# eladhoffer/convNet.pytorch

Hardware: NVIDIA H100
Metric: ResNet-50 images/sec (training step, synthetic 224x224) (higher is better)
Workload: dtype bf16

## Files before the change

convnet/pytorch_b200/csrc/conv.cu:

```cuda
#include "common.cuh"
#include "host.h"
#include <stdlib.h>
#include <utility>

namespace b200 {

constexpr int kMaxStages = 8;
constexpr int kMaxTaps = 32;
constexpr int kThreads = 384;
constexpr int kConsumers = 256;
constexpr int kProducerWarp = 8;
constexpr int kTileM = 128;
constexpr int kStatReplicas = 16;

struct TapEntry {
  uint16_t off_w, off_h;
  uint16_t b_tap;
  uint16_t pad_;
};

struct IgemmParams {
  int M_total;
  int I, J;
  int trav;
// ... 749 lines not shown
            "smem=%d\n",
            p.M_total, L.SC, L.Nout, L.ntaps, L.os, p.block_n, p.n_tiles, p.m_tiles, p.ck, L.ntaps * p.c_chunks,
            p.num_stages, p.tma_store, p.plain_a, p.b_stationary, p.own_ntile, p.out_fp32, L.bias != nullptr,
            L.res != nullptr, p.act, L.stats != nullptr, grid, max_tiles, smem_bytes);
  }
  b200::launch(kfn, grid, kThreads, smem_bytes, stream, tmA, tmB, tmC, tmR, p);
  B200_CHECK_LAUNCH("conv_igemm_kernel");
  return B200_OK;
}

static int check_desc(const b200_conv_desc* d) {
  B200_REQUIRE(d != nullptr, B200_ERR_INVALID, "conv: null descriptor");
  B200_REQUIRE(d->N > 0 && d->H > 0 && d->W > 0 && d->C > 0 && d->K > 0 && d->R > 0 && d->S > 0 && d->P > 0 &&
                   d->Q > 0 && d->stride >= 1 && d->stride <= 8,
               B200_ERR_INVALID, "conv: bad descriptor N=%d H=%d W=%d C=%d K=%d R=%d S=%d P=%d Q=%d stride=%d", d->N,
               d->H, d->W, d->C, d->K, d->R, d->S, d->P, d->Q, d->stride);
  B200_REQUIRE(d->R * d->S <= kMaxTaps, B200_ERR_UNSUPPORTED, "conv: %dx%d filter exceeds %d taps", d->R, d->S,
               kMaxTaps);
  B200_REQUIRE((d->x_pixel_stride == 0 && d->x_row_stride == 0 && d->x_image_stride == 0) ||
                   (d->x_pixel_stride > 0 && d->x_pixel_stride % 8 == 0 && d->x_row_stride % 8 == 0 &&
                    d->x_image_stride % 8 == 0 && d->x_row_stride > 0 && d->x_image_stride > 0),
               B200_ERR_INVALID, "conv: x strides must all be 0 (dense) or positive multiples of 8 elements");
  B200_REQUIRE(d->window == 0 || (d->window % 64 == 0 && d->C == d->K && d->C % d->window == 0 && d->x_pixel_stride == 0),
               B200_ERR_UNSUPPORTED, "conv: window %d needs C == K, C %% window == 0 (C=%d K=%d)", d->window, d->C, d->K);
  return B200_OK;
}

}

using namespace b200;

extern "C" int b200_conv_fprop(const b200_conv_desc* d, const void* x, const void* w, void* y,
                               const b200_epilogue* ep, b200_stream_t stream) {
  int rc = check_desc(d);
  if (rc) return rc;
  B200_REQUIRE(x && w && y, B200_ERR_INVALID, "conv_fprop: null pointer");
  B200_REQUIRE(d->C % 8 == 0, B200_ERR_UNSUPPORTED, "conv_fprop: C=%d must be a multiple of 8 (pad the input)", d->C);
  if (d->stride == 1 && d->pad_h == d->pad_w && d->P == d->H + 2 * d->pad_h - d->R + 1 &&
      d->Q == d->W + 2 * d->pad_w - d->S + 1 && d->x_pixel_stride == 0 && (!ep || !ep->out_fp32) &&
      !(ep && ep->bias && ep->bn_stats_workspace) && (d->window == 0 || d->window == 64) &&
      halo_eligible(d->P, d->Q, d->C, d->K, d->R, d->S, d->pad_h)) {
    return launch_halo(x, w, y, ep ? ep->residual : nullptr, ep ? ep->bias : nullptr, d->N, d->P, d->Q, d->C, d->K,
                       d->R, d->S, d->pad_h, 0, ep ? ep->act : 0,
                       (ep && ep->bn_stats_workspace) ? reinterpret_cast<double*>(ep->bn_stats_workspace) : nullptr,
                       (cudaStream_t)stream, d->window);
  }
  IgemmLaunch L;
  memset(&L, 0, sizeof(L));
  L.src = x; L.Nimg = d->N; L.SH = d->H; L.SW = d->W; L.SC = d->C;
  L.s_pix = d->x_pixel_stride; L.s_row = d->x_row_stride; L.s_img = d->x_image_stride;
  L.wmat = w; L.Nout = d->K; L.wtaps = d->R * d->S;
  L.I = d->P; L.J = d->Q; L.trav = d->stride; L.lower_w = -d->pad_w; L.lower_h = -d->pad_h;
  L.ntaps = d->R * d->S;
  for (int r = 0; r < d->R; ++r)
    for (int s = 0; s < d->S; ++s) {
      TapEntry& t = L.taps[r * d->S + s];
      t.off_w = (uint16_t)s; t.off_h = (uint16_t)r; t.b_tap = (uint16_t)(r * d->S + s); t.pad_ = 0;
    }
  L.out = y; L.OH = d->P; L.OW = d->Q; L.os = 1; L.oh0 = 0; L.ow0 = 0; L.ldo = d->K;
  L.res = ep ? ep->residual : nullptr;
  L.bias = ep ? ep->bias : nullptr;
  L.act = ep ? ep->act : 0;
  L.out_fp32 = ep ? ep->out_fp32 : 0;
  L.stats = (ep && ep->bn_stats_workspace) ? reinterpret_cast<double*>(ep->bn_stats_workspace) : nullptr;
  L.window = d->window;
  return launch_igemm(L, (cudaStream_t)stream);
}

extern "C" int b200_conv_dgrad(const b200_conv_desc* d, const void* dy, const void* wt, void* dx,
                               const void* residual, b200_stream_t stream_) {
  int rc = check_desc(d);
  if (rc) return rc;
  cudaStream_t stream = (cudaStream_t)stream_;
  B200_REQUIRE(dy && wt && dx, B200_ERR_INVALID, "conv_dgrad: null pointer");
  B200_REQUIRE(d->K % 8 == 0, B200_ERR_UNSUPPORTED, "conv_dgrad: K=%d must be a multiple of 8", d->K);
  const int st = d->stride;
  B200_REQUIRE(st == 1 || st == 2, B200_ERR_UNSUPPORTED, "conv_dgrad: stride %d unsupported", st);
  if (d->R == 3 && d->S == 3 && st == 1 && d->pad_h == 1 && d->pad_w == 1 && d->P == d->H && d->Q == d->W &&
      (d->window == 0 || d->window == 64) && halo_eligible(d->H, d->W, d->K, d->C, 3, 3, 1)) {
    return launch_halo(dy, wt, dx, residual, nullptr, d->N, d->H, d->W, d->K, d->C, 3, 3, 1, 1, 0, nullptr, stream,
                       d->window);
  }
  bool any_empty = false;
  for (int ph = 0; ph < st; ++ph)
    for (int pw = 0; pw < st; ++pw) {
      int nr = 0, ns = 0;
      for (int r = 0; r < d->R; ++r) if (((ph + d->pad_h - r) % st + st) % st == 0) ++nr;
      for (int s = 0; s < d->S; ++s) if (((pw + d->pad_w - s) % st + st) % st == 0) ++ns;
      if (nr * ns == 0 && (d->H - ph + st - 1) / st > 0 && (d->W - pw + st - 1) / st > 0) any_empty = true;
    }
  if (any_empty) {
    B200_REQUIRE(residual == nullptr, B200_ERR_UNSUPPORTED,
                 "conv_dgrad: residual add with an empty stride class is unsupported");
    cudaError_t e = cudaMemsetAsync(dx, 0, (size_t)d->N * d->H * d->W * d->C * 2, stream);
    B200_REQUIRE(e == cudaSuccess, B200_ERR_CUDA, "conv_dgrad: memset failed: %s", cudaGetErrorString(e));
    count_launch();
  }
  for (int ph = 0; ph < st; ++ph)
    for (int pw = 0; pw < st; ++pw) {
      const int I = (d->H - ph + st - 1) / st;
      const int J = (d->W - pw + st - 1) / st;
      if (I <= 0 || J <= 0) continue;
      IgemmLaunch L;
      memset(&L, 0, sizeof(L));
      int dh[kMaxTaps], dwv[kMaxTaps], rr[kMaxTaps], ss[kMaxTaps];
      int nr = 0, ns = 0;
      for (int r = 0; r < d->R; ++r) {
        const int v = ph + d->pad_h - r;
        if (((v % st) + st) % st == 0) { dh[nr] = (v - (((v % st) + st) % st)) / st; rr[nr] = r; ++nr; }
      }
      for (int s = 0; s < d->S; ++s) {
        const int v = pw + d->pad_w - s;
        if (((v % st) + st) % st == 0) { dwv[ns] = (v - (((v % st) + st) % st)) / st; ss[ns] = s; ++ns; }
      }
      if (nr * ns == 0) continue;
      int lo_h = dh[0], lo_w = dwv[0];
      for (int i = 1; i < nr; ++i) lo_h = dh[i] < lo_h ? dh[i] : lo_h;
      for (int i = 1; i < ns; ++i) lo_w = dwv[i] < lo_w ? dwv[i] : lo_w;
      L.ntaps = nr * ns;
      for (int a = 0; a < nr; ++a)
        for (int b = 0; b < ns; ++b) {
          TapEntry& t = L.taps[a * ns + b];
          t.off_h = (uint16_t)(dh[a] - lo_h);
          t.off_w = (uint16_t)(dwv[b] - lo_w);
          t.b_tap = (uint16_t)(rr[a] * d->S + ss[b]);
          t.pad_ = 0;
        }
      L.src = dy; L.Nimg = d->N; L.SH = d->P; L.SW = d->Q; L.SC = d->K;
      L.wmat = wt; L.Nout = d->C; L.wtaps = d->R * d->S;
      L.I = I; L.J = J; L.trav = 1; L.lower_w = lo_w; L.lower_h = lo_h;
      L.out = dx; L.OH = d->H; L.OW = d->W; L.os = st; L.oh0 = ph; L.ow0 = pw; L.ldo = d->C;
      L.res = residual; L.bias = nullptr; L.act = 0; L.out_fp32 = 0;
      L.window = d->window;
      rc = launch_igemm(L, stream);
      if (rc) return rc;
    }
  return B200_OK;
}

extern "C" size_t b200_conv_wgrad_workspace_bytes(void) {
  return static_cast<size_t>(sm_count() + 8) * kTileM * 512 * sizeof(float);
}

extern "C" int b200_conv_wgrad(const b200_conv_desc* d, const void* x, const void* dy, float* dw, void* workspace,
                               size_t workspace_bytes, b200_stream_t stream_) {
  int rc = check_desc(d);
  if (rc) return rc;
  cudaStream_t stream = (cudaStream_t)stream_;
  B200_REQUIRE(x && dy && dw, B200_ERR_INVALID, "conv_wgrad: null pointer");
  B200_REQUIRE(d->C % 8 == 0 && d->K % 8 == 0, B200_ERR_UNSUPPORTED,
               "conv_wgrad: C=%d and K=%d must be multiples of 8", d->C, d->K);
  if (d->stride == 1 && d->pad_h == d->pad_w && d->P == d->H + 2 * d->pad_h - d->R + 1 &&
      d->Q == d->W + 2 * d->pad_w - d->S + 1 && d->x_pixel_stride == 0 &&
      (d->window == 0 || d->window == 128) && halo_wgrad_eligible(d->P, d->Q, d->C, d->K, d->R, d->S, d->pad_h)) {
    const int units = ((d->window ? d->window : d->C) / 16) * ((d->K + kTileM - 1) / kTileM);
    if (units <= sm_count() + 8)
      return launch_halo_wgrad(x, dy, dw, workspace, workspace_bytes, d->N, d->P, d->Q, d->C, d->K, d->R, d->S, d->pad_h,
                               stream, d->window);
  }
  B200_REQUIRE(d->window == 0 || d->window == 128, B200_ERR_UNSUPPORTED, "conv_wgrad: window must be 0 or 128");
  const int Cw = d->window ? d->window : d->C;
  WgradParams p;
  memset(&p, 0, sizeof(p));
  p.M_total = d->N * d->P * d->Q;
  p.P = d->P; p.Q = d->Q; p.trav = d->stride; p.lower_w = -d->pad_w; p.lower_h = -d->pad_h;
  p.K_out = d->K; p.C = Cw; p.taps_total = d->R * d->S;
  p.window = d->window;
  p.ckA = pick_ck(d->K);
  p.ckB = pick_ck(Cw);
  p.bk = kBk;
  p.c_chunks = (Cw + p.ckB - 1) / p.ckB;
  p.total_boxes = p.taps_total * p.c_chunks;
  p.k_tiles = (d->K + kTileM - 1) / kTileM;
  p.boxA_bytes = p.bk * p.ckA * 2;
  p.boxB_bytes = p.bk * p.ckB * 2;
  p.kt = 1;
  p.boxes_per_cta = 256 / p.ckB;
  if (p.boxes_per_cta > 8) p.boxes_per_cta = 8;
  if (p.boxes_per_cta > p.total_boxes) p.boxes_per_cta = p.total_boxes;
  p.k_groups = (p.k_tiles + p.kt - 1) / p.kt;
  p.col_groups = (p.total_boxes + p.boxes_per_cta - 1) / p.boxes_per_cta;
  p.total_blocks = (p.M_total + p.bk - 1) / p.bk;
  const int tiles = p.k_groups * p.col_groups;
  int splits = sm_count() / tiles;
  if (splits > p.total_blocks) splits = p.total_blocks;
  if (splits < 1) splits = 1;
  p.blocks_per_split = (p.total_blocks + splits - 1) / splits;
  p.splits = (p.total_blocks + p.blocks_per_split - 1) / p.blocks_per_split;
  p.stage_bytes = p.kt * (kTileM / p.ckA) * p.boxA_bytes + p.boxes_per_cta * p.boxB_bytes;
  p.stage_bytes = (p.stage_bytes + 1023u) & ~1023u;
  p.num_stages = kSmemBudget / (int)p.stage_bytes;
  if (p.num_stages > kMaxStages) p.num_stages = kMaxStages;
  if (p.num_stages < 2) p.num_stages = 2;
  p.dw = dw;
  p.pitch = p.kt * p.boxes_per_cta * p.ckB;
  p.partial = nullptr;
  if (p.splits > 1) {
    const size_t need = static_cast<size_t>(tiles) * p.splits * kTileM * p.pitch * sizeof(float);
    B200_REQUIRE(workspace != nullptr && workspace_bytes >= need, B200_ERR_INVALID,
                 "conv_wgrad: workspace too small (%zu < %zu); see b200_conv_wgrad_workspace_bytes()", workspace_bytes,
                 need);
    B200_REQUIRE((Cw & 3) == 0, B200_ERR_UNSUPPORTED, "conv_wgrad: C must be a multiple of 4");
    p.partial = static_cast<float*>(workspace);
  }
  p.S_filter = d->S;
  CUtensorMap tmDy, tmX;
  rc = encode_tiled2(&tmDy, dy, d->K, (long long)p.M_total, p.ckA, p.bk);
  if (rc) return rc;
  const int upper_w = p.lower_w + (d->Q - 1) * d->stride + 1 - d->W;
  const int upper_h = p.lower_h + (d->P - 1) * d->stride + 1 - d->H;
  p.plain_x = (d->R == 1 && d->S == 1 && d->stride == 1 && d->pad_h == 0 && d->pad_w == 0 && d->P == d->H &&
               d->Q == d->W && d->x_pixel_stride == 0) ? 1 : 0;
  if (getenv("B200_WGRAD_DEBUG"))
    fprintf(stderr, "[wgrad] K=%d C=%d taps=%d stride=%d ckA=%d ckB=%d kt=%d bpc=%d k_groups=%d col_groups=%d splits=%d "
            "bps=%d stages=%d stage=%u nc=%d nboxes_last=%d plain_x=%d partial=%d\n", d->K, d->C, p.taps_total,
            d->stride, p.ckA, p.ckB, p.kt, p.boxes_per_cta, p.k_groups, p.col_groups, p.splits, p.blocks_per_split,
            p.num_stages, p.stage_bytes, p.pitch, p.total_boxes - (p.col_groups - 1) * p.boxes_per_cta, p.plain_x,
            p.partial != nullptr);
  if (p.plain_x)
    rc = encode_tiled2(&tmX, x, d->C, (long long)p.M_total, p.ckB, p.bk);
  else
    rc = encode_im2col(&tmX, x, d->N, d->H, d->W, d->C, p.ckB, p.bk, p.lower_w, p.lower_h, upper_w, upper_h,
                       d->stride, d->x_pixel_stride, d->x_row_stride, d->x_image_stride);
  if (rc) return rc;
  const int smem_bytes = p.num_stages * (int)p.stage_bytes + 1024;
  const auto kfn = wgrad_kernel_for(p.pitch, std::make_integer_sequence<int, 16>{});
  rc = set_smem_attr((const void*)kfn, smem_bytes);
  if (rc) return rc;
  const int grid = tiles * p.splits;
  b200::launch(kfn, grid, kThreads, smem_bytes, stream, tmDy, tmX, p);
  B200_CHECK_LAUNCH("conv_wgrad_kernel");
  if (p.partial != nullptr) {
    const long long total = static_cast<long long>(d->K) * p.taps_total * (Cw / 4);
    long long blocks = (total + 31) / 32;
    if (blocks > 16LL * sm_count()) blocks = 16LL * sm_count();
    b200::launch(conv_wgrad_reduce_kernel, static_cast<int>(blocks), 32 * wgrad_reduce_warps(p.splits), 0, stream, p.partial, dw, d->K, p.taps_total, Cw, p.ckB,
                                                                          p.c_chunks, p.boxes_per_cta, p.kt, p.k_groups,
                                                                          p.splits, p.pitch);
    B200_CHECK_LAUNCH("conv_wgrad_reduce_kernel");
  }
  return B200_OK;
}
```

convnet/pytorch_b200/csrc/conv3x3.cu:

```cuda
#include "common.cuh"
#include "host.h"
#include <stdlib.h>

namespace b200 {

constexpr int kHThreads = 384;
constexpr int kHTileM = 128;
constexpr int kHMaxA = 6, kHMaxB = 8;
constexpr int kHMaxTaps = 16;
constexpr int kHStatReplicas = 16;

struct HaloParams {
  int N, H, W, C, Kout;
  int RT, Wp;
  int tiles_per_img, m_tiles, n_tiles, block_n, c_chunks;
  int sa, sb;
  uint32_t a_bytes, a_box_bytes, b_bytes;
  int act;
  int has_res;
  double* stats;
  const float* bias;
  int ntaps, pad;
  int row_bytes;
  int b_stationary;
  int diag;
  uint16_t a_off[kHMaxTaps];
  uint16_t b_tap[kHMaxTaps];
};

template <int NTAPS, int KSTEPS, int BN>
__global__ void __launch_bounds__(kHThreads, 1)
conv_halo_kernel(const __grid_constant__ CUtensorMap tmX, const __grid_constant__ CUtensorMap tmB,
                 const __grid_constant__ CUtensorMap tmC, const __grid_constant__ CUtensorMap tmR,
                 const __grid_constant__ HaloParams p) {
  extern __shared__ uint8_t smem_raw[];
  __shared__ __align__(8) uint64_t a_full[kHMaxA], a_empty[kHMaxA], b_full[kHMaxB], b_empty[kHMaxB];
  __shared__ __align__(8) uint64_t res_bar, bstat_bar;

  const int warp = threadIdx.x >> 5, lane = threadIdx.x & 31;
  const uint32_t raw_addr = smem_u32(smem_raw);
  uint8_t* smem = smem_raw + (((raw_addr + 1023u) & ~1023u) - raw_addr);
  uint8_t* sA = smem;
  uint8_t* sB = sA + p.sa * p.a_bytes;
  const int b_slots = p.b_stationary ? p.c_chunks * p.ntaps : p.sb;
  uint8_t* epi = sB + b_slots * p.b_bytes;

  if (threadIdx.x == 0) {
    for (int i = 0; i < p.sa; ++i) { mbar_init(&a_full[i], 1); mbar_init(&a_empty[i], 8); }
    for (int i = 0; i < kHMaxB; ++i) { mbar_init(&b_full[i], 1); mbar_init(&b_empty[i], 8); }
    mbar_init(&bstat_bar, 1);
    mbar_init(&res_bar, 1);
    fence_mbar_init();
    prefetch_tmap(&tmX); prefetch_tmap(&tmB); prefetch_tmap(&tmC);
    if (p.has_res) prefetch_tmap(&tmR);
  }
  __syncthreads();
  pdl_wait();
  const int t_start = p.diag ? static_cast<int>(blockIdx.x) / p.n_tiles : static_cast<int>(blockIdx.x);
  const int t_step = p.diag ? static_cast<int>(gridDim.x) / p.n_tiles : static_cast<int>(gridDim.x);
  const int total_tiles = p.diag ? p.m_tiles : p.m_tiles * p.n_tiles;
  const int own_n = static_cast<int>(blockIdx.x) % p.n_tiles;

  if (warp >= 8) {
    producer_setmaxnreg();
    if (warp == 8 && lane == 0) {
      int ia = 0, ib = 0; uint32_t pa = 0, pb = 0;
      const int cw = p.row_bytes >> 1;
      if (p.b_stationary && t_start < total_tiles) {
        mbar_arrive_expect_tx(&bstat_bar, static_cast<uint32_t>(p.c_chunks * NTAPS) * p.b_bytes);
        for (int cc = 0; cc < p.c_chunks; ++cc)
          for (int t = 0; t < NTAPS; ++t)
            tma_load_3d(&tmB, &bstat_bar, sB + (cc * NTAPS + t) * p.b_bytes, cc * cw, p.b_tap[t],
                        p.diag ? own_n * p.block_n : 0);
      }
      for (int tile = t_start; tile < total_tiles; tile += t_step) {
        const int m_tile = p.diag ? tile : tile / p.n_tiles, n_tile = p.diag ? own_n : tile - m_tile * p.n_tiles;
        const int img = m_tile / p.tiles_per_img;
        const int h0 = (m_tile - img * p.tiles_per_img) * p.RT;
        for (int cc = 0; cc < p.c_chunks; ++cc) {
          mbar_wait(&a_empty[ia], pa ^ 1u);
          mbar_arrive_expect_tx(&a_full[ia], p.a_box_bytes);
          tma_load_4d(&tmX, &a_full[ia], sA + ia * p.a_bytes, (p.diag ? n_tile : cc) * cw, -p.pad, h0 - p.pad, img);
          if (++ia == p.sa) { ia = 0; pa ^= 1u; }
          if (p.b_stationary) continue;
          for (int t = 0; t < NTAPS; ++t) {
            mbar_wait(&b_empty[ib], pb ^ 1u);
            mbar_arrive_expect_tx(&b_full[ib], p.b_bytes);
            tma_load_3d(&tmB, &b_full[ib], sB + ib * p.b_bytes, cc * cw, p.b_tap[t], n_tile * p.block_n);
            if (++ib == p.sb) { ib = 0; pb ^= 1u; }
          }
        }
      }
    }
    return;
  }
  consumer_setmaxnreg();

  const int wg = warp >> 2;
  const int r_lo = wg * 64 + (warp & 3) * 16 + (lane >> 2);
  const int c_lo = 2 * (lane & 3);
  const bool leader = threadIdx.x == 0;
  const uint64_t proto = make_smem_desc(0, 16, 8u * p.row_bytes, layout_type_for_row_bytes(p.row_bytes));
  const uint32_t a_wg = (64u * wg * p.row_bytes) >> 4;
  const int nbox = BN >> 6;
  const uint32_t box_bytes = static_cast<uint32_t>(p.RT * p.W) * 128u;
  const uint32_t box_pitch = (box_bytes + 1023u) & ~1023u;
  int srow[2];
  bool in_tile[2];
#pragma unroll
  for (int h = 0; h < 2; ++h) {
    const int v = r_lo + 8 * h;
    const int ry = v / p.Wp, cx = v - ry * p.Wp;
    srow[h] = ry * p.W + cx;
    in_tile[h] = (ry < p.RT) && (cx < p.W);
  }
  const int st_col = threadIdx.x % BN;
  const int st_rows = kHTileM / (256 / BN);
  const int st_row0 = (threadIdx.x / BN) * st_rows;
  int st_ntile = -1;
  float st_s1 = 0.f, st_s2 = 0.f;
  if (p.b_stationary && t_start < total_tiles) mbar_wait(&bstat_bar, 0);

  float acc[BN / 2];
  int ia = 0, ib = 0; uint32_t pa = 0, pb = 0;
  int local = 0;
  for (int tile = t_start; tile < total_tiles; tile += t_step, ++local) {
    const int m_tile = p.diag ? tile : tile / p.n_tiles, n_tile = p.diag ? own_n : tile - m_tile * p.n_tiles;
    const int img = m_tile / p.tiles_per_img;
    const int h0 = (m_tile - img * p.tiles_per_img) * p.RT;
    const int nbase = n_tile * BN;
    if (leader && local > 0) bulk_wait_group_read0();
    named_bar_sync(1, 256);
    if (leader && p.has_res) {
      fence_proxy_async();
      mbar_arrive_expect_tx(&res_bar, static_cast<uint32_t>(nbox) * box_bytes);
      for (int b = 0; b < nbox; ++b) tma_load_4d(&tmR, &res_bar, epi + b * box_pitch, nbase + b * 64, 0, h0, img);
    }

    wgmma_fence_acc(acc);
    int rel_a = -1, rel_b = -1;
    for (int cc = 0; cc < p.c_chunks; ++cc) {
      mbar_wait(&a_full[ia], pa);
      const uint64_t da0 = proto + (smem_u32(sA + ia * p.a_bytes) >> 4) + a_wg;
#pragma unroll
      for (int t = 0; t < NTAPS; ++t) {
        uint64_t db0;
        if (p.b_stationary) {
          db0 = proto + (smem_u32(sB + (cc * NTAPS + t) * p.b_bytes) >> 4);
        } else {
          mbar_wait(&b_full[ib], pb);
          db0 = proto + (smem_u32(sB + ib * p.b_bytes) >> 4);
        }
        const uint32_t tap_inc = (static_cast<uint32_t>(p.a_off[t]) * p.row_bytes) >> 4;
        wgmma_fence();
#pragma unroll
        for (int k = 0; k < KSTEPS; ++k)
          wgmma_bf16<0, 0>(acc, da0 + tap_inc + 2 * k, db0 + 2 * k, (cc | t | k) != 0 ? 1u : 0u);
        if (!p.b_stationary || t == NTAPS - 1) {
          wgmma_commit();
          wgmma_wait<1>();
          if (rel_b >= 0) release_stage(&b_empty[rel_b], lane);
          if (rel_a >= 0) release_stage(&a_empty[rel_a], lane);
          rel_a = (t == NTAPS - 1) ? ia : -1;
          rel_b = p.b_stationary ? -1 : ib;
        }
        if (!p.b_stationary && ++ib == p.sb) { ib = 0; pb ^= 1u; }
      }
      if (++ia == p.sa) { ia = 0; pa ^= 1u; }
    }
    wgmma_wait<0>();
    wgmma_fence_acc(acc);
    if (rel_b >= 0) release_stage(&b_empty[rel_b], lane);
    if (rel_a >= 0) release_stage(&a_empty[rel_a], lane);

    if (p.has_res) mbar_wait(&res_bar, static_cast<uint32_t>(local & 1));
#pragma unroll
    for (int h = 0; h < 2; ++h) {
      if (!in_tile[h] || h0 + (r_lo + 8 * h) / p.Wp >= p.H) continue;
      const int row = srow[h];
#pragma unroll
      for (int j = 0; j < BN / 2; j += 4) {
        const int c = 2 * j + c_lo;
        {
          uint32_t* dst = reinterpret_cast<uint32_t*>(epi + (c >> 6) * box_pitch + row * 128 +
                                                      ((((c & 63) >> 3) ^ (row & 7)) << 4) + (c & 7) * 2);
          float v0 = acc[j + 2 * h], v1 = acc[j + 2 * h + 1];
          if (p.bias != nullptr) { v0 += __ldg(p.bias + nbase + c); v1 += __ldg(p.bias + nbase + c + 1); }
          if (p.has_res) {
            const float2 t2 = unpack_bf16x2(*dst);
            v0 += t2.x;
            v1 += t2.y;
          }
          *dst = pack_bf16x2(apply_act(v0, p.act), apply_act(v1, p.act));
        }
      }
    }
    fence_proxy_async();
    named_bar_sync(1, 256);
    if (leader) {
      for (int b = 0; b < nbox; ++b) tma_store_4d(&tmC, epi + b * box_pitch, nbase + b * 64, 0, h0, img);
      bulk_commit_group();
    }
    if (p.stats != nullptr) {
      if (st_ntile != n_tile) {
        if (st_ntile >= 0) {
          double* dst = p.stats + (blockIdx.x % kHStatReplicas) * 2 * p.Kout + st_ntile * BN + st_col;
          atomicAdd(dst, (double)st_s1);
          atomicAdd(dst + p.Kout, (double)st_s2);
        }
        st_ntile = n_tile; st_s1 = 0.f; st_s2 = 0.f;
      }
      const int vrows = min(p.RT, p.H - h0) * p.W;
      const uint8_t* col = epi + (st_col >> 6) * box_pitch + (st_col & 7) * 2;
      const int j = (st_col & 63) >> 3;
      const int r_end = min(st_row0 + st_rows, vrows);
      for (int r = st_row0; r < r_end; ++r) {
        const float x = __bfloat162float(*reinterpret_cast<const __nv_bfloat16*>(col + r * 128 + ((j ^ (r & 7)) << 4)));
        st_s1 += x;
        st_s2 = fmaf(x, x, st_s2);
      }
    }
  }
  if (p.stats != nullptr && st_ntile >= 0) {
    double* dst = p.stats + (blockIdx.x % kHStatReplicas) * 2 * p.Kout + st_ntile * BN + st_col;
    atomicAdd(dst, (double)st_s1);
    atomicAdd(dst + p.Kout, (double)st_s2);
  }
  if (leader) bulk_wait_group0();
}

typedef void (*HaloKernelFn)(const __grid_constant__ CUtensorMap, const __grid_constant__ CUtensorMap,
                             const __grid_constant__ CUtensorMap, const __grid_constant__ CUtensorMap,
                             const __grid_constant__ HaloParams);
static HaloKernelFn halo_kernel_for(int ntaps, int block_n) {
  if (ntaps == 9)
    return block_n == 64 ? conv_halo_kernel<9, 4, 64> : block_n == 128 ? conv_halo_kernel<9, 4, 128>
         : block_n == 256 ? conv_halo_kernel<9, 4, 256> : nullptr;
  if (ntaps == 16)
    return block_n == 64 ? conv_halo_kernel<16, 1, 64> : block_n == 128 ? conv_halo_kernel<16, 1, 128>
         : block_n == 256 ? conv_halo_kernel<16, 1, 256> : nullptr;
  return nullptr;
}

static int enc4(CUtensorMap* tm, const void* base, int C, int W, int H, int N, int b0, int b1, int b2) {
  EncodeTiledFn fn = encode_tiled_fn();
  B200_REQUIRE(fn != nullptr, B200_ERR_CUDA, "cuTensorMapEncodeTiled entry point unavailable");
  cuuint64_t dims[4] = {(cuuint64_t)C, (cuuint64_t)W, (cuuint64_t)H, (cuuint64_t)N};
  cuuint64_t strides[3] = {(cuuint64_t)C * 2, (cuuint64_t)W * C * 2, (cuuint64_t)H * W * C * 2};
  cuuint32_t box[4] = {(cuuint32_t)b0, (cuuint32_t)b1, (cuuint32_t)b2, 1};
  cuuint32_t es[4] = {1, 1, 1, 1};
  CUresult r = fn(tm, CU_TENSOR_MAP_DATA_TYPE_BFLOAT16, 4, const_cast<void*>(base), dims, strides, box, es,
                  CU_TENSOR_MAP_INTERLEAVE_NONE, swizzle_for_row_bytes(b0 * 2), CU_TENSOR_MAP_L2_PROMOTION_L2_128B,
                  CU_TENSOR_MAP_FLOAT_OOB_FILL_NONE);
  B200_REQUIRE(r == CUDA_SUCCESS, B200_ERR_CUDA, "cuTensorMapEncodeTiled(4d) failed (%d) dims=(%d,%d,%d,%d) box=(%d,%d,%d)",
               (int)r, C, W, H, N, b0, b1, b2);
  return B200_OK;
}

static bool halo_enabled() {
  static const bool enabled = !(getenv("B200_HALO") && atoi(getenv("B200_HALO")) == 0);
  return enabled;
}

bool halo_geometry_ok(int H, int W, int Cs, int R, int S, int pad) {
  if (!halo_enabled()) return false;
  const bool k3 = (R == 3 && S == 3 && pad == 1 && Cs % 64 == 0);
  const bool k4 = (R == 4 && S == 4 && pad == 0 && Cs == 16);
  if (!k3 && !k4) return false;
  const int Wp = W + S - 1;
  if (Wp > 128 || W < 8) return false;
  int RT = 128 / Wp;
  if (RT > H) RT = H;
  const int tiles = (H + RT - 1) / RT;
  return (double)H * W / (128.0 * tiles) >= 0.6;
}

bool halo_eligible(int H, int W, int Cs, int Nout, int R, int S, int pad) {
  if (!halo_geometry_ok(H, W, Cs, R, S, pad) || Nout % 64 != 0) return false;
  const int n_tiles = (Nout + 255) / 256;
  const int block_n = Nout / n_tiles;
  return Nout % n_tiles == 0 && block_n % 64 == 0 && 256 % block_n == 0;
}

int launch_halo(const void* src, const void* wmat, void* out, const void* res, const float* bias, int N, int H, int W,
                int Cs, int Nout, int R, int S, int pad, int dir, int act, double* stats, cudaStream_t stream, int window) {
  HaloParams p;
  memset(&p, 0, sizeof(p));
  p.diag = window > 0 ? 1 : 0;
  if (p.diag)
    B200_REQUIRE(window == 64 && Cs == Nout && Cs % 64 == 0 && R == 3 && S == 3, B200_ERR_UNSUPPORTED,
                 "conv halo: window mode needs window == 64, C == K, C %% 64 == 0 and a 3x3 filter (C=%d K=%d)", Cs, Nout);
  p.N = N; p.H = H; p.W = W; p.C = Cs; p.Kout = Nout;
  p.ntaps = R * S; p.pad = pad;
  p.row_bytes = (Cs == 16) ? 32 : 128;
  const int cw = p.row_bytes / 2;
  p.Wp = W + S - 1;
  p.RT = 128 / p.Wp;
  if (p.RT > H) p.RT = H;
  p.tiles_per_img = (H + p.RT - 1) / p.RT;
  p.m_tiles = N * p.tiles_per_img;
  p.n_tiles = p.diag ? Nout / 64 : (Nout + 255) / 256;
  p.block_n = Nout / p.n_tiles;
  p.c_chunks = p.diag ? 1 : Cs / cw;
  p.a_box_bytes = (uint32_t)(p.RT + R - 1) * p.Wp * p.row_bytes;
  uint32_t a_need = (uint32_t)(kHTileM + (R - 1) * p.Wp + (S - 1)) * p.row_bytes;
  if (a_need < p.a_box_bytes) a_need = p.a_box_bytes;
  p.a_bytes = (a_need + 1023u) & ~1023u;
  p.b_bytes = (uint32_t)p.block_n * p.row_bytes;
  p.act = act;
  p.has_res = res != nullptr;
  p.stats = stats;
  p.bias = bias;
  for (int r = 0; r < R; ++r)
    for (int s = 0; s < S; ++s) {
      const int t = r * S + s;
      p.b_tap[t] = (uint16_t)t;
      p.a_off[t] = (uint16_t)(dir == 0 ? r * p.Wp + s : (R - 1 - r) * p.Wp + (S - 1 - s));
    }
  const uint32_t box_pitch = (((uint32_t)(p.RT * W) * 128u) + 1023u) & ~1023u;
  const uint32_t epi_bytes = (uint32_t)(p.block_n / 64) * box_pitch;
  int budget = 212 * 1024 - (int)epi_bytes;
  const int b_all = p.c_chunks * p.ntaps * (int)p.b_bytes;
  p.b_stationary = ((p.n_tiles == 1 || p.diag) && b_all <= 80 * 1024) ? 1 : 0;
  B200_REQUIRE(!p.diag || p.b_stationary, B200_ERR_UNSUPPORTED, "conv halo: window mode expects resident weights");
  int b_region;
  if (p.b_stationary) {
    b_region = b_all;
    p.sb = 0;
    p.sa = (budget - b_region) / (int)p.a_bytes;
    if (p.sa > kHMaxA) p.sa = kHMaxA;
  } else {
    p.sa = 2;
    p.sb = (budget - p.sa * (int)p.a_bytes) / (int)p.b_bytes;
    if (p.sb > kHMaxB) p.sb = kHMaxB;
    if (p.sb >= 6 && (int)(3 * p.a_bytes + 4 * p.b_bytes) <= budget) {
      p.sa = 3;
      p.sb = (budget - 3 * (int)p.a_bytes) / (int)p.b_bytes;
      if (p.sb > kHMaxB) p.sb = kHMaxB;
    }
    b_region = p.sb * (int)p.b_bytes;
  }
  B200_REQUIRE(p.sa >= 2 && (p.b_stationary || p.sb >= 2), B200_ERR_UNSUPPORTED,
               "conv halo: shared memory budget exceeded (W=%d, block_n=%d)", W, p.block_n);
  CUtensorMap tmX, tmB, tmC, tmR;
  memset(&tmR, 0, sizeof(tmR));
  int rc = enc4(&tmX, src, Cs, W + S - 1 - 2 * pad, H + R - 1 - 2 * pad, N, cw, p.Wp, p.RT + R - 1);
  if (rc) return rc;
  {
    EncodeTiledFn fn = encode_tiled_fn();
    const int wc = p.diag ? window : Cs;
    cuuint64_t dims[3] = {(cuuint64_t)wc, (cuuint64_t)p.ntaps, (cuuint64_t)Nout};
    cuuint64_t strides[2] = {(cuuint64_t)wc * 2, (cuuint64_t)wc * p.ntaps * 2};
    cuuint32_t box[3] = {(cuuint32_t)cw, 1, (cuuint32_t)p.block_n};
    cuuint32_t es[3] = {1, 1, 1};
    CUresult r = fn(&tmB, CU_TENSOR_MAP_DATA_TYPE_BFLOAT16, 3, const_cast<void*>(wmat), dims, strides, box, es,
                    CU_TENSOR_MAP_INTERLEAVE_NONE, swizzle_for_row_bytes(p.row_bytes),
                    CU_TENSOR_MAP_L2_PROMOTION_L2_128B, CU_TENSOR_MAP_FLOAT_OOB_FILL_NONE);
    B200_REQUIRE(r == CUDA_SUCCESS, B200_ERR_CUDA, "conv halo: weight tensor map failed (%d)", (int)r);
  }
  rc = enc4(&tmC, out, Nout, W, H, N, 64, W, p.RT);
  if (rc) return rc;
  if (res) {
    rc = enc4(&tmR, res, Nout, W, H, N, 64, W, p.RT);
    if (rc) return rc;
  }
  const int smem_bytes = p.sa * (int)p.a_bytes + b_region + (int)epi_bytes + 1024;
  HaloKernelFn kfn = halo_kernel_for(p.ntaps, p.block_n);
  B200_REQUIRE(kfn != nullptr, B200_ERR_UNSUPPORTED, "conv halo: %d taps with block_n %d unsupported", p.ntaps, p.block_n);
  cudaError_t e = cudaFuncSetAttribute((const void*)kfn, cudaFuncAttributeMaxDynamicSharedMemorySize, smem_bytes);
  B200_REQUIRE(e == cudaSuccess, B200_ERR_CUDA, "conv halo: smem attribute (%d bytes): %s", smem_bytes, cudaGetErrorString(e));
  const int total = p.m_tiles * p.n_tiles;
  int grid = total < sm_count() ? total : sm_count();
  if (p.diag) {
    int per_n = sm_count() / p.n_tiles;
    if (per_n > p.m_tiles) per_n = p.m_tiles;
    if (per_n < 1) per_n = 1;
    grid = per_n * p.n_tiles;
  }
  if (getenv("B200_HALO_DEBUG"))
    fprintf(stderr, "[halo] dir=%d N=%d H=%d W=%d C=%d K=%d taps=%d block_n=%d n_tiles=%d m_tiles=%d bstat=%d diag=%d "
            "sa=%d sb=%d bias=%d res=%d act=%d stats=%d grid=%d\n", dir, N, H, W, Cs, Nout, p.ntaps, p.block_n,
            p.n_tiles, p.m_tiles, p.b_stationary, p.diag, p.sa, p.sb, bias != nullptr, res != nullptr, act,
            stats != nullptr, grid);
  b200::launch(kfn, grid, kHThreads, smem_bytes, stream, tmX, tmB, tmC, tmR, p);
  B200_CHECK_LAUNCH("conv_halo_kernel");
  return B200_OK;
}


constexpr int kWThreads = 384;
constexpr int kWMaxStages = 4;

struct HaloWgradParams {
  int N, H, W, K_out, C;
  int RT, Wp, tiles_per_img, m_tiles;
  int ntaps, pad, halo_rows;
  int x_row_bytes, cw, ncols;
  int c_chunks, k_tiles, units, splits, tiles_per_split;
  int stages;
  int window;
  uint32_t a_box_bytes, a_bytes, x_box_bytes, x_bytes;
  float* partial;
  uint16_t x_off[kHMaxTaps];
};

template <int R, int S>
__global__ void __launch_bounds__(kWThreads, 1)
conv_halo_wgrad_kernel(const __grid_constant__ CUtensorMap tmDy, const __grid_constant__ CUtensorMap tmX,
                       const __grid_constant__ HaloWgradParams p) {
  constexpr int kCols = S * 16;
  extern __shared__ uint8_t smem_raw[];
  __shared__ __align__(8) uint64_t full_bar[kWMaxStages], empty_bar[kWMaxStages];
  const int warp = threadIdx.x >> 5, lane = threadIdx.x & 31;
  const uint32_t raw_addr = smem_u32(smem_raw);
  uint8_t* smem = smem_raw + (((raw_addr + 1023u) & ~1023u) - raw_addr);
  const uint32_t stage_bytes = p.a_bytes + p.x_bytes;

  {
    uint4* z = reinterpret_cast<uint4*>(smem);
    const int n16 = static_cast<int>(p.stages * stage_bytes) >> 4;
    for (int i = threadIdx.x; i < n16; i += kWThreads) z[i] = make_uint4(0u, 0u, 0u, 0u);
  }
  if (threadIdx.x == 0) {
    for (int s = 0; s < p.stages; ++s) { mbar_init(&full_bar[s], 1); mbar_init(&empty_bar[s], 8); }
    fence_mbar_init();
    prefetch_tmap(&tmDy);
    prefetch_tmap(&tmX);
  }
  fence_proxy_async();
  __syncthreads();
  pdl_wait();

  const int split = blockIdx.x / p.units;
  const int unit = blockIdx.x - split * p.units;
  const int k_tile = unit % p.k_tiles;
  const int cc = unit / p.k_tiles;
  const int k0 = k_tile * kHTileM;
  const int t_begin = split * p.tiles_per_split;
  const int t_end = min(p.m_tiles, t_begin + p.tiles_per_split);
  const int ntiles = t_end - t_begin;
  const int nA = min(2, (p.K_out - k0 + 63) / 64);
  if (ntiles <= 0) return;

  if (warp >= 8) {
    producer_setmaxnreg();
    if (warp == 8 && lane == 0) {
      int stage = 0; uint32_t phase = 0;
      const uint32_t tx = nA * p.a_box_bytes + p.x_box_bytes;
      for (int tile = t_begin; tile < t_end; ++tile) {
        const int img = tile / p.tiles_per_img;
        const int h0 = (tile - img * p.tiles_per_img) * p.RT;
        mbar_wait(&empty_bar[stage], phase ^ 1u);
        uint8_t* sa = smem + stage * stage_bytes;
        mbar_arrive_expect_tx(&full_bar[stage], tx);
        for (int j = 0; j < nA; ++j) tma_load_4d(&tmDy, &full_bar[stage], sa + j * 16384, k0 + j * 64, 0, h0, img);
        tma_load_4d(&tmX, &full_bar[stage], sa + p.a_bytes, cc * p.cw + (p.window ? k0 : 0), -p.pad, h0 - p.pad, img);
        if (++stage == p.stages) { stage = 0; phase ^= 1u; }
      }
    }
    return;
  }
  consumer_setmaxnreg();

  const int wg = warp >> 2;
  const bool wg_on = wg < nA;
  const uint64_t protoA = make_smem_desc(0, 16384, 1024, 1);
  const uint64_t protoX = make_smem_desc(0, p.x_row_bytes, 8u * p.x_row_bytes, layout_type_for_row_bytes(p.x_row_bytes));
  uint32_t row_inc[R];
#pragma unroll
  for (int r = 0; r < R; ++r) row_inc[r] = (static_cast<uint32_t>(p.x_off[r * S]) * p.x_row_bytes) >> 4;
  const uint32_t kx_inc = (16u * p.x_row_bytes) >> 4;
  float acc[R][kCols / 2];
#pragma unroll
  for (int r = 0; r < R; ++r) wgmma_fence_acc(acc[r]);
  int stage = 0, prev = 0; uint32_t phase = 0;
  for (int i = 0; i < ntiles; ++i) {
    mbar_wait(&full_bar[stage], phase);
    if (wg_on) {
      const uint32_t a_addr = smem_u32(smem + stage * stage_bytes);
      const uint64_t da0 = protoA + ((a_addr + wg * 16384) >> 4);
      const uint64_t dx0 = protoX + ((a_addr + p.a_bytes) >> 4);
      wgmma_fence();
#pragma unroll
      for (int k = 0; k < 8; ++k) {
        const uint32_t scale = (k != 0 || i != 0) ? 1u : 0u;
#pragma unroll
        for (int r = 0; r < R; ++r)
          wgmma_bf16<1, 1>(acc[r], da0 + k * 128, dx0 + row_inc[r] + k * kx_inc, scale);
      }
      wgmma_commit();
      wgmma_wait<1>();
    }
    if (i > 0) release_stage(&empty_bar[prev], lane);
    prev = stage;
    if (++stage == p.stages) { stage = 0; phase ^= 1u; }
  }
  wgmma_wait<0>();
#pragma unroll
  for (int r = 0; r < R; ++r) wgmma_fence_acc(acc[r]);
  release_stage(&empty_bar[prev], lane);
  if (!wg_on) return;

  const int row = wg * 64 + (warp & 3) * 16 + (lane >> 2);
  const int c_lo = 2 * (lane & 3);
#pragma unroll
  for (int h = 0; h < 2; ++h) {
    float* dst = p.partial + ((static_cast<long long>(unit) * p.splits + split) * kHTileM + row + 8 * h) * p.ncols;
#pragma unroll
    for (int r = 0; r < R; ++r)
#pragma unroll
      for (int j = 0; j < kCols / 2; j += 4)
        *reinterpret_cast<float2*>(dst + r * kCols + 2 * j + c_lo) = make_float2(acc[r][j + 2 * h], acc[r][j + 2 * h + 1]);
  }
}

__global__ void __launch_bounds__(256) conv_halo_wgrad_reduce_kernel(const float* __restrict__ partial,
                                                                     float* __restrict__ dw, int K_out, int ntaps, int C,
                                                                     int cw, int k_tiles, int splits, int ncols) {
  pdl_wait();
  __shared__ float4 red[8][32];
  const int c4n = C >> 2;
  const long long total = static_cast<long long>(K_out) * ntaps * c4n;
  const int lane = threadIdx.x & 31, w = threadIdx.x >> 5, nw = blockDim.x >> 5;
  for (long long base = static_cast<long long>(blockIdx.x) * 32; base < total; base += static_cast<long long>(gridDim.x) * 32) {
    const long long idx = base + lane;
    float4 acc = make_float4(0.f, 0.f, 0.f, 0.f);
    int c = 0, tap = 0, k = 0;
    if (idx < total) {
      c = static_cast<int>(idx % c4n) * 4;
      tap = static_cast<int>((idx / c4n) % ntaps);
      k = static_cast<int>(idx / (static_cast<long long>(c4n) * ntaps));
      const int k_tile = k >> 7, row = k & 127;
      const int cc = c / cw;
      const int unit = cc * k_tiles + k_tile;
      const float* src = partial + ((static_cast<long long>(unit) * splits) * kHTileM + row) * ncols + tap * cw + (c - cc * cw);
      for (int s2 = w; s2 < splits; s2 += nw) {
        const float4 v = __ldcg(reinterpret_cast<const float4*>(src + static_cast<long long>(s2) * kHTileM * ncols));
        acc.x += v.x; acc.y += v.y; acc.z += v.z; acc.w += v.w;
      }
    }
    red[w][lane] = acc;
    __syncthreads();
    if (w == 0 && idx < total) {
      for (int j = 1; j < nw; ++j) {
        const float4 v = red[j][lane];
        acc.x += v.x; acc.y += v.y; acc.z += v.z; acc.w += v.w;
      }
      float4* d = reinterpret_cast<float4*>(dw + (static_cast<long long>(k) * ntaps + tap) * C + c);
      float4 o = *d;
      o.x += acc.x; o.y += acc.y; o.z += acc.z; o.w += acc.w;
      *d = o;
    }
    __syncthreads();
  }
}

bool halo_wgrad_eligible(int H, int W, int C, int K_out, int R, int S, int pad) {
  static const bool enabled = !(getenv("B200_HALO_WGRAD") && atoi(getenv("B200_HALO_WGRAD")) == 0);
  if (!enabled || !halo_geometry_ok(H, W, C, R, S, pad)) return false;
  return K_out % 64 == 0;
}

int launch_halo_wgrad(const void* x, const void* dy, float* dw, void* workspace, size_t workspace_bytes, int N, int H,
                      int W, int C, int K_out, int R, int S, int pad, cudaStream_t stream, int window) {
  HaloWgradParams p;
  memset(&p, 0, sizeof(p));
  p.window = window;
  if (window)
    B200_REQUIRE(window == 128 && C == K_out && C % 128 == 0, B200_ERR_UNSUPPORTED,
                 "conv halo wgrad: window mode needs window == 128 and C == K, C %% 128 == 0 (C=%d K=%d)", C, K_out);
  p.N = N; p.H = H; p.W = W; p.K_out = K_out; p.C = C;
  p.ntaps = R * S; p.pad = pad;
  p.cw = 16;
  p.x_row_bytes = p.cw * 2;
  p.ncols = p.ntaps * p.cw;
  p.Wp = W + S - 1;
  p.RT = 128 / p.Wp;
  if (p.RT > H) p.RT = H;
  p.halo_rows = p.RT + R - 1;
  p.tiles_per_img = (H + p.RT - 1) / p.RT;
  p.m_tiles = N * p.tiles_per_img;
  p.c_chunks = (window ? window : C) / p.cw;
  p.k_tiles = (K_out + kHTileM - 1) / kHTileM;
  p.units = p.c_chunks * p.k_tiles;
  int splits = sm_count() / p.units;
  if (splits < 1) splits = 1;
  if (splits > p.m_tiles) splits = p.m_tiles;
  p.tiles_per_split = (p.m_tiles + splits - 1) / splits;
  p.splits = (p.m_tiles + p.tiles_per_split - 1) / p.tiles_per_split;
  p.a_box_bytes = (uint32_t)(p.RT * p.Wp) * 128u;
  p.a_bytes = 2 * 16384;
  p.x_box_bytes = (uint32_t)(p.halo_rows * p.Wp) * p.x_row_bytes;
  int max_off = 0;
  for (int r = 0; r < R; ++r)
    for (int s = 0; s < S; ++s) {
      p.x_off[r * S + s] = (uint16_t)(r * p.Wp + s);
      if (r * p.Wp + s > max_off) max_off = r * p.Wp + s;
    }
  uint32_t x_need = (uint32_t)(kHTileM + max_off) * p.x_row_bytes;
  if (x_need < p.x_box_bytes) x_need = p.x_box_bytes;
  p.x_bytes = (x_need + 1023u) & ~1023u;
  p.stages = (212 * 1024) / (int)(p.a_bytes + p.x_bytes);
  if (p.stages > kWMaxStages) p.stages = kWMaxStages;
  B200_REQUIRE(p.stages >= 2, B200_ERR_UNSUPPORTED, "conv halo wgrad: shared memory budget exceeded (W=%d)", W);
  const size_t need = (size_t)p.units * p.splits * kHTileM * p.ncols * sizeof(float);
  B200_REQUIRE(workspace != nullptr && workspace_bytes >= need, B200_ERR_INVALID,
               "conv halo wgrad: workspace of %zu bytes needed (%zu given)", need, workspace_bytes);
  p.partial = reinterpret_cast<float*>(workspace);
  CUtensorMap tmDy, tmX;
  int rc = enc4(&tmDy, dy, K_out, W, H, N, 64, p.Wp, p.RT);
  if (rc) return rc;
  rc = enc4(&tmX, x, C, W + S - 1 - 2 * pad, H + R - 1 - 2 * pad, N, p.cw, p.Wp, p.halo_rows);
  if (rc) return rc;
  const int smem_bytes = p.stages * (int)(p.a_bytes + p.x_bytes) + 1024;
  const void* kfn = (p.ntaps == 9) ? (const void*)conv_halo_wgrad_kernel<3, 3> : (const void*)conv_halo_wgrad_kernel<4, 4>;
  cudaError_t e = cudaFuncSetAttribute(kfn, cudaFuncAttributeMaxDynamicSharedMemorySize, smem_bytes);
  B200_REQUIRE(e == cudaSuccess, B200_ERR_CUDA, "conv halo wgrad: smem attribute (%d bytes): %s", smem_bytes,
               cudaGetErrorString(e));
  if (getenv("B200_HALO_DEBUG"))
    fprintf(stderr, "[halo_wgrad] N=%d H=%d W=%d C=%d K=%d taps=%d k_tiles=%d c_chunks=%d m_tiles=%d units=%d "
            "splits=%d tiles_per_split=%d stages=%d grid=%d\n", N, H, W, C, K_out, p.ntaps, p.k_tiles, p.c_chunks,
            p.m_tiles, p.units, p.splits, p.tiles_per_split, p.stages, p.units * p.splits);
  if (p.ntaps == 9)
    b200::launch(conv_halo_wgrad_kernel<3, 3>, p.units * p.splits, kWThreads, smem_bytes, stream, tmDy, tmX, p);
  else
    b200::launch(conv_halo_wgrad_kernel<4, 4>, p.units * p.splits, kWThreads, smem_bytes, stream, tmDy, tmX, p);
  B200_CHECK_LAUNCH("conv_halo_wgrad_kernel");
  const int Cw = window ? window : C;
  const long long total = (long long)K_out * p.ntaps * (Cw / 4);
  long long blocks64 = (total + 31) / 32;
  if (blocks64 > 16LL * sm_count()) blocks64 = 16LL * sm_count();
  const int blocks = (int)blocks64;
  b200::launch(conv_halo_wgrad_reduce_kernel, blocks, 32 * wgrad_reduce_warps(p.splits), 0, stream, p.partial, dw, K_out, p.ntaps, Cw, p.cw, p.k_tiles, p.splits,
                                                            p.ncols);
  B200_CHECK_LAUNCH("conv_halo_wgrad_reduce_kernel");
  return B200_OK;
}

}
```

convnet/pytorch_b200/csrc/host.h:

```cpp
#pragma once
#include <cuda.h>
#include <cuda_runtime.h>
#include <stdarg.h>
#include <stdio.h>
#include "../../../include/b200conv.h"

namespace b200 {

void set_error(const char* fmt, ...);
void count_launch(int n = 1);
int sm_count();

typedef CUresult (*EncodeTiledFn)(CUtensorMap*, CUtensorMapDataType, cuuint32_t, void*, const cuuint64_t*,
                                  const cuuint64_t*, const cuuint32_t*, const cuuint32_t*, CUtensorMapInterleave,
                                  CUtensorMapSwizzle, CUtensorMapL2promotion, CUtensorMapFloatOOBfill);
typedef CUresult (*EncodeIm2colFn)(CUtensorMap*, CUtensorMapDataType, cuuint32_t, void*, const cuuint64_t*,
                                   const cuuint64_t*, const int*, const int*, cuuint32_t, cuuint32_t,
                                   const cuuint32_t*, CUtensorMapInterleave, CUtensorMapSwizzle,
                                   CUtensorMapL2promotion, CUtensorMapFloatOOBfill);
EncodeTiledFn encode_tiled_fn();
EncodeIm2colFn encode_im2col_fn();

bool halo_geometry_ok(int H, int W, int Cs, int R, int S, int pad);
bool halo_eligible(int H, int W, int Cs, int Nout, int R, int S, int pad);
int launch_halo(const void* src, const void* wmat, void* out, const void* res, const float* bias, int N, int H, int W,
                int Cs, int Nout, int R, int S, int pad, int dir, int act, double* stats, cudaStream_t stream,
                int window = 0);

bool halo_wgrad_eligible(int H, int W, int C, int K_out, int R, int S, int pad);
int launch_halo_wgrad(const void* x, const void* dy, float* dw, void* workspace, size_t workspace_bytes, int N, int H,
                      int W, int C, int K_out, int R, int S, int pad, cudaStream_t stream, int window = 0);

bool pdl_enabled();
template <typename... KArgs, typename... Args>
inline void launch(void (*kernel)(KArgs...), dim3 grid, dim3 block, size_t smem, cudaStream_t stream, Args&&... args) {
  cudaLaunchConfig_t cfg = {};
  cfg.gridDim = grid;
  cfg.blockDim = block;
  cfg.dynamicSmemBytes = smem;
  cfg.stream = stream;
  cudaLaunchAttribute attr[1];
  attr[0].id = cudaLaunchAttributeProgrammaticStreamSerialization;
  attr[0].val.programmaticStreamSerializationAllowed = 1;
  cfg.attrs = attr;
  cfg.numAttrs = pdl_enabled() ? 1 : 0;
  cudaLaunchKernelEx(&cfg, kernel, static_cast<KArgs>(args)...);
}

int wgrad_reduce_warps(int splits);

inline CUtensorMapSwizzle swizzle_for_row_bytes(int row_bytes) {
  return row_bytes == 128 ? CU_TENSOR_MAP_SWIZZLE_128B
                          : (row_bytes == 64 ? CU_TENSOR_MAP_SWIZZLE_64B : CU_TENSOR_MAP_SWIZZLE_32B);
}

#define B200_CHECK_LAUNCH(name)                                                   \
  do {                                                                            \
    cudaError_t e__ = cudaGetLastError();                                         \
    if (e__ != cudaSuccess) {                                                     \
      b200::set_error("%s: launch failed: %s", name, cudaGetErrorString(e__));    \
      return B200_ERR_CUDA;                                                       \
    }                                                                             \
    b200::count_launch();                                                         \
  } while (0)

#define B200_REQUIRE(cond, code, ...)   \
  do {                                  \
    if (!(cond)) {                      \
      b200::set_error(__VA_ARGS__);     \
      return code;                      \
    }                                   \
  } while (0)

}
```

Measured before the change: 5510.

## Widen halo wgrad channel tile for 3x3 and specialize stationary-B MMA loop

For 3x3 weight-gradient convolutions the halo kernel now uses a 32-channel x-tile instead of 16, which halves the number of work units per K tile and doubles the columns each CTA computes per dy load. The eligibility check, including the unit-count limit, moves into halo_wgrad_eligible so that it uses the new tile width. This lets more layers take the halo wgrad path. The forward halo kernel also specializes its MMA chunk loop at compile time on b_stationary, and in stationary mode it issues the wgmma fence only on the first tap. The wider tile raises shared memory and register pressure per stage and gives fewer CTAs for small-C layers.

Result: faster. 5620, median of 6 (+2.0%).

```diff
diff --git a/convnet/pytorch_b200/csrc/conv.cu b/convnet/pytorch_b200/csrc/conv.cu
--- a/convnet/pytorch_b200/csrc/conv.cu
+++ b/convnet/pytorch_b200/csrc/conv.cu
@@ -925,12 +925,10 @@
                "conv_wgrad: C=%d and K=%d must be multiples of 8", d->C, d->K);
   if (d->stride == 1 && d->pad_h == d->pad_w && d->P == d->H + 2 * d->pad_h - d->R + 1 &&
       d->Q == d->W + 2 * d->pad_w - d->S + 1 && d->x_pixel_stride == 0 &&
-      (d->window == 0 || d->window == 128) && halo_wgrad_eligible(d->P, d->Q, d->C, d->K, d->R, d->S, d->pad_h)) {
-    const int units = ((d->window ? d->window : d->C) / 16) * ((d->K + kTileM - 1) / kTileM);
-    if (units <= sm_count() + 8)
-      return launch_halo_wgrad(x, dy, dw, workspace, workspace_bytes, d->N, d->P, d->Q, d->C, d->K, d->R, d->S, d->pad_h,
-                               stream, d->window);
-  }
+      (d->window == 0 || d->window == 128) &&
+      halo_wgrad_eligible(d->P, d->Q, d->C, d->K, d->R, d->S, d->pad_h, d->window))
+    return launch_halo_wgrad(x, dy, dw, workspace, workspace_bytes, d->N, d->P, d->Q, d->C, d->K, d->R, d->S, d->pad_h,
+                             stream, d->window);
   B200_REQUIRE(d->window == 0 || d->window == 128, B200_ERR_UNSUPPORTED, "conv_wgrad: window must be 0 or 128");
   const int Cw = d->window ? d->window : d->C;
   WgradParams p;
diff --git a/convnet/pytorch_b200/csrc/conv3x3.cu b/convnet/pytorch_b200/csrc/conv3x3.cu
--- a/convnet/pytorch_b200/csrc/conv3x3.cu
+++ b/convnet/pytorch_b200/csrc/conv3x3.cu
@@ -1,6 +1,7 @@
 #include "common.cuh"
 #include "host.h"
 #include <stdlib.h>
+#include <type_traits>
 
 namespace b200 {
 
@@ -139,34 +140,39 @@
 
     wgmma_fence_acc(acc);
     int rel_a = -1, rel_b = -1;
-    for (int cc = 0; cc < p.c_chunks; ++cc) {
+    auto chunk_mmas = [&](int cc, auto stationary) {
+      constexpr bool kStat = decltype(stationary)::value;
       mbar_wait(&a_full[ia], pa);
       const uint64_t da0 = proto + (smem_u32(sA + ia * p.a_bytes) >> 4) + a_wg;
 #pragma unroll
       for (int t = 0; t < NTAPS; ++t) {
         uint64_t db0;
-        if (p.b_stationary) {
+        if constexpr (kStat) {
           db0 = proto + (smem_u32(sB + (cc * NTAPS + t) * p.b_bytes) >> 4);
         } else {
           mbar_wait(&b_full[ib], pb);
           db0 = proto + (smem_u32(sB + ib * p.b_bytes) >> 4);
         }
         const uint32_t tap_inc = (static_cast<uint32_t>(p.a_off[t]) * p.row_bytes) >> 4;
-        wgmma_fence();
+        if (!kStat || t == 0) wgmma_fence();
 #pragma unroll
         for (int k = 0; k < KSTEPS; ++k)
           wgmma_bf16<0, 0>(acc, da0 + tap_inc + 2 * k, db0 + 2 * k, (cc | t | k) != 0 ? 1u : 0u);
-        if (!p.b_stationary || t == NTAPS - 1) {
+        if (!kStat || t == NTAPS - 1) {
           wgmma_commit();
           wgmma_wait<1>();
           if (rel_b >= 0) release_stage(&b_empty[rel_b], lane);
           if (rel_a >= 0) release_stage(&a_empty[rel_a], lane);
           rel_a = (t == NTAPS - 1) ? ia : -1;
-          rel_b = p.b_stationary ? -1 : ib;
+          rel_b = kStat ? -1 : ib;
         }
-        if (!p.b_stationary && ++ib == p.sb) { ib = 0; pb ^= 1u; }
+        if (!kStat && ++ib == p.sb) { ib = 0; pb ^= 1u; }
       }
       if (++ia == p.sa) { ia = 0; pa ^= 1u; }
+    };
+    for (int cc = 0; cc < p.c_chunks; ++cc) {
+      if (p.b_stationary) chunk_mmas(cc, std::true_type{});
+      else chunk_mmas(cc, std::false_type{});
     }
     wgmma_wait<0>();
     wgmma_fence_acc(acc);
@@ -404,11 +410,11 @@
   uint16_t x_off[kHMaxTaps];
 };
 
-template <int R, int S>
+template <int R, int S, int CW>
 __global__ void __launch_bounds__(kWThreads, 1)
 conv_halo_wgrad_kernel(const __grid_constant__ CUtensorMap tmDy, const __grid_constant__ CUtensorMap tmX,
                        const __grid_constant__ HaloWgradParams p) {
-  constexpr int kCols = S * 16;
+  constexpr int kCols = S * CW;
   extern __shared__ uint8_t smem_raw[];
   __shared__ __align__(8) uint64_t full_bar[kWMaxStages], empty_bar[kWMaxStages];
   const int warp = threadIdx.x >> 5, lane = threadIdx.x & 31;
@@ -555,10 +561,13 @@
   }
 }
 
-bool halo_wgrad_eligible(int H, int W, int C, int K_out, int R, int S, int pad) {
+static int halo_wgrad_cw(int R) { return R == 3 ? 32 : 16; }
+
+bool halo_wgrad_eligible(int H, int W, int C, int K_out, int R, int S, int pad, int window) {
   static const bool enabled = !(getenv("B200_HALO_WGRAD") && atoi(getenv("B200_HALO_WGRAD")) == 0);
-  if (!enabled || !halo_geometry_ok(H, W, C, R, S, pad)) return false;
-  return K_out % 64 == 0;
+  if (!enabled || !halo_geometry_ok(H, W, C, R, S, pad) || K_out % 64 != 0) return false;
+  const int units = ((window ? window : C) / halo_wgrad_cw(R)) * ((K_out + kHTileM - 1) / kHTileM);
+  return units <= sm_count() + 8;
 }
 
 int launch_halo_wgrad(const void* x, const void* dy, float* dw, void* workspace, size_t workspace_bytes, int N, int H,
@@ -571,7 +580,7 @@
                  "conv halo wgrad: window mode needs window == 128 and C == K, C %% 128 == 0 (C=%d K=%d)", C, K_out);
   p.N = N; p.H = H; p.W = W; p.K_out = K_out; p.C = C;
   p.ntaps = R * S; p.pad = pad;
-  p.cw = 16;
+  p.cw = halo_wgrad_cw(R);
   p.x_row_bytes = p.cw * 2;
   p.ncols = p.ntaps * p.cw;
   p.Wp = W + S - 1;
@@ -613,7 +622,8 @@
   rc = enc4(&tmX, x, C, W + S - 1 - 2 * pad, H + R - 1 - 2 * pad, N, p.cw, p.Wp, p.halo_rows);
   if (rc) return rc;
   const int smem_bytes = p.stages * (int)(p.a_bytes + p.x_bytes) + 1024;
-  const void* kfn = (p.ntaps == 9) ? (const void*)conv_halo_wgrad_kernel<3, 3> : (const void*)conv_halo_wgrad_kernel<4, 4>;
+  const void* kfn = (p.ntaps == 9) ? (const void*)conv_halo_wgrad_kernel<3, 3, 32>
+                                   : (const void*)conv_halo_wgrad_kernel<4, 4, 16>;
   cudaError_t e = cudaFuncSetAttribute(kfn, cudaFuncAttributeMaxDynamicSharedMemorySize, smem_bytes);
   B200_REQUIRE(e == cudaSuccess, B200_ERR_CUDA, "conv halo wgrad: smem attribute (%d bytes): %s", smem_bytes,
                cudaGetErrorString(e));
@@ -622,9 +632,9 @@
             "splits=%d tiles_per_split=%d stages=%d grid=%d\n", N, H, W, C, K_out, p.ntaps, p.k_tiles, p.c_chunks,
             p.m_tiles, p.units, p.splits, p.tiles_per_split, p.stages, p.units * p.splits);
   if (p.ntaps == 9)
-    b200::launch(conv_halo_wgrad_kernel<3, 3>, p.units * p.splits, kWThreads, smem_bytes, stream, tmDy, tmX, p);
+    b200::launch(conv_halo_wgrad_kernel<3, 3, 32>, p.units * p.splits, kWThreads, smem_bytes, stream, tmDy, tmX, p);
   else
-    b200::launch(conv_halo_wgrad_kernel<4, 4>, p.units * p.splits, kWThreads, smem_bytes, stream, tmDy, tmX, p);
+    b200::launch(conv_halo_wgrad_kernel<4, 4, 16>, p.units * p.splits, kWThreads, smem_bytes, stream, tmDy, tmX, p);
   B200_CHECK_LAUNCH("conv_halo_wgrad_kernel");
   const int Cw = window ? window : C;
   const long long total = (long long)K_out * p.ntaps * (Cw / 4);
diff --git a/convnet/pytorch_b200/csrc/host.h b/convnet/pytorch_b200/csrc/host.h
--- a/convnet/pytorch_b200/csrc/host.h
+++ b/convnet/pytorch_b200/csrc/host.h
@@ -27,7 +27,7 @@
                 int Cs, int Nout, int R, int S, int pad, int dir, int act, double* stats, cudaStream_t stream,
                 int window = 0);
 
-bool halo_wgrad_eligible(int H, int W, int C, int K_out, int R, int S, int pad);
+bool halo_wgrad_eligible(int H, int W, int C, int K_out, int R, int S, int pad, int window);
 int launch_halo_wgrad(const void* x, const void* dy, float* dw, void* workspace, size_t workspace_bytes, int N, int H,
                       int W, int C, int K_out, int R, int S, int pad, cudaStream_t stream, int window = 0);
 
```
